# pj8912/python-p2p-network

Hardware: AMD Instinct MI355X
Metric: msg-edge relays/sec (GTEPS) at 10M peers x 4096 msgs; % HBM roofline (higher is better)
Workload: dtype u64

## Files before the change

python-p2p-network_amd/csrc/relay_kernels.hip:

```cpp
#include <hip/hip_runtime.h>

#include <algorithm>
#include <cstdlib>
#include <cstring>
#include <type_traits>

#include "device_util.h"

#ifndef P2PG_PICK_DIRECT
#define P2PG_PICK_DIRECT 1
#endif
#ifndef P2PG_PICK_FOLD
#define P2PG_PICK_FOLD 1
#endif


namespace p2pg {
namespace {

__global__ void k_zero_rows(uint64_t* plane, int32_t W, const int32_t* rows, int32_t n) {
  const int64_t i = (int64_t)blockIdx.x * blockDim.x + threadIdx.x;
  if (i >= (int64_t)n * W) return;
  const int64_t r = rows[i / W];
  if (r < 0) return;
  plane[r * W + (i % W)] = 0ull;
}

__global__ void k_seed(DevState st, const int32_t* src, int32_t M) {
  const int m = blockIdx.x * blockDim.x + threadIdx.x;
  if (m >= M) return;
  const int64_t v = src[m];
  if (v < 0) return;
  const uint64_t bit = 1ull << (m & 63);
  const int64_t o = v * st.W + (m >> 6);
  atomicOr((unsigned long long*)&st.F[0][o], (unsigned long long)bit);
  atomicOr((unsigned long long*)&st.seen[o], (unsigned long long)bit);
  atomicOr(&st.A[0][v >> 5], 1u << (v & 31));
  if (st.AW[0]) atomicOr((unsigned long long*)&st.AW[0][v], 1ull << (m >> 6));
}

template <bool CHURN, bool GOSSIP>
__global__ __launch_bounds__(256) void k_pull(DevGraph g, DevState st, RoundParams p) {
  const int lane = threadIdx.x & 63;
  const int wib = wave_in_block();
  const int64_t V = g.V;
  const int W = st.W;
  const int cur = p.round & 1, prv = cur ^ 1;
  const uint64_t* __restrict__ Src = GOSSIP ? st.E[prv] : st.F[prv];
  uint64_t* __restrict__ Fc = st.F[cur];
  const uint32_t* __restrict__ Ap = st.A[prv];
  const int64_t ntasks = (V + 31) >> 5;
  const int nslices = (W + 63) >> 6;
  uint64_t c[STAT_N] = {0, 0, 0, 0, 0, 0, 0, 0};

  for (int64_t task = (int64_t)blockIdx.x * WPB + wib; task < ntasks;
       task += (int64_t)gridDim.x * WPB) {
    const int64_t u0 = task << 5;
    const uint32_t sat0 = st.S[task];
    uint32_t sat = sat0;
    uint32_t todo = ~sat0 & phase_mask(p, task);
    if (V - u0 < 32) todo &= (1u << (V - u0)) - 1u;
    uint32_t aw = 0;
    while (todo) {
      const int b = __builtin_ctz(todo);
      todo &= todo - 1u;
      const int64_t u = u0 + b;
      const int64_t beg = g.rowptr[u], end = g.rowptr[u + 1];
      const uint64_t deg = (uint64_t)(end - beg);
      const uint64_t per_bit = GOSSIP ? (deg < (uint64_t)p.fanout ? deg : (uint64_t)p.fanout)
                                      : deg - 1;
      bool row_new = false, row_full = true;
      for (int sl = 0; sl < nslices; ++sl) {
        const int w = sl * 64 + lane;
        const bool valid = w < W;
        const uint64_t fm = valid ? full_mask(w, W, st.M) : 0ull;
        const uint64_t s = valid ? st.seen[u * W + w] : 0ull;
        const uint64_t need = fm & ~s;
        uint64_t acc = 0;
        if (__ballot(need != 0ull)) {
          for (int64_t cb = beg; cb < end; cb += 64) {
            const int64_t j = cb + lane;
            uint32_t srow = 0;
            bool act = false;
            if (j < end) {
              const int32_t v = g.colidx[j];
              act = bit_test(Ap, v);
              if (CHURN && act)
                act = !churn_dropped((uint32_t)(p.round - 1), gidx(g, u), gidx(g, v),
                                     p.churn_thr, p.cseed_lo, p.cseed_hi);
              srow = GOSSIP ? (uint32_t)j : (uint32_t)v;
            }
            uint64_t m = __ballot(act);
            while (m) {
              uint32_t sv[8];
              bool ok[8];
#pragma unroll
              for (int k = 0; k < 8; ++k) {
                ok[k] = m != 0ull;
                if (m) {
                  const int idx = __builtin_ctzll(m);
                  m &= m - 1ull;
                  sv[k] = (uint32_t)__builtin_amdgcn_readlane((int)srow, idx);
                } else {
                  sv[k] = 0u;
                }
              }
              uint64_t x[8];
#pragma unroll
              for (int k = 0; k < 8; ++k)
                x[k] = (ok[k] && need) ? Src[(int64_t)sv[k] * W + w] : 0ull;
#pragma unroll
              for (int k = 0; k < 8; ++k) acc |= x[k];
            }
          }
        }
        const uint64_t nw = acc & need;
        const bool any = __ballot(nw != 0ull) != 0ull;
        row_new |= any;
        if (__ballot(valid && (s | nw) != fm)) row_full = false;
        if (nw) st_prow(&st.seen[u * W + w], s | nw);
        if (valid && (any || nslices > 1)) st_prow(&Fc[u * W + w], nw);
        if (nw) {
          const uint64_t pc = (uint64_t)__popcll(nw);
          c[ST_NEW] += pc;
          c[ST_RELAYS] += pc * per_bit;
          c[ST_ACTIVE_W] += 1;
          c[ST_WEDGES] += deg;
        }
      }
      if (row_new) {
        aw |= 1u << b;
        if (lane == 0) {
          c[ST_ACTIVE_V] += 1;
          c[ST_DEG_ACT] += deg;
        }
      }
      if (row_full) sat |= 1u << b;
    }
    if (lane == 0) {
      put_active(st.A[cur], task, aw, p);
      if (sat != sat0) st.S[task] = sat;
    }
  }
  flush_stats(st.stats, c, lane);
}


struct PullStage {
  int b;
  int64_t beg, end;
  uint64_t s;
  int32_t v;
  uint32_t r;
  bool act;
  uint32_t aword;
  uint64_t mr;
  uint64_t am;
  uint32_t rv;
};

__device__ __forceinline__ bool aw_has(const uint64_t* __restrict__ AW, int64_t v, int w) {
  return !AW || ((ldc(AW + v) >> w) & 1ull);
}

struct FusedStage {
  int32_t u;
  uint32_t beg, end;
  uint64_t s;
  int32_t v;
  uint32_t aword;
  uint64_t mr;
  uint64_t am;
  uint32_t rv;
};

__device__ __forceinline__ uint64_t src_word(const uint64_t* __restrict__ Src, uint32_t row,
                                             int W, int lane, bool packed, uint64_t am,
                                             bool want) {
  if (!packed) return want ? at_row(Src, row, W)[lane] : 0ull;
  const bool here = want && ((am >> lane) & 1ull);
  const int pos = __popcll(am & ((1ull << lane) - 1ull));
  return here ? at_row(Src, row, W)[pos] : 0ull;
}


__device__ __forceinline__ uint64_t src_word_m(const uint64_t* __restrict__ Src, uint32_t row,
                                               int W, uint64_t am, uint64_t h) {
  uint64_t x = 0ull;
  if (__builtin_amdgcn_inverse_ballot_w64(h)) {
    const uint32_t pos = __builtin_amdgcn_mbcnt_hi((uint32_t)(am >> 32),
                                                   __builtin_amdgcn_mbcnt_lo((uint32_t)am, 0u));
#if P2PG_NT_LOADS
    x = __builtin_nontemporal_load(at_row(Src, row, W) + pos);
#else
    x = at_row(Src, row, W)[pos];
#endif
  }
  return x;
}

__device__ __forceinline__ uint64_t src_word_pair(const uint64_t* __restrict__ Src, uint32_t r0,
                                                  uint32_t r1, int W, uint32_t m0, uint32_t m1,
                                                  uint32_t h0, uint32_t h1) {
  uint64_t x = 0ull;
  if (__builtin_amdgcn_inverse_ballot_w64((uint64_t)h0 | ((uint64_t)h1 << 32))) {
    const bool lo = __builtin_amdgcn_mbcnt_hi(~0u, __builtin_amdgcn_mbcnt_lo(~0u, 0u)) < 32u;
    const uint32_t pos = __builtin_amdgcn_mbcnt_hi(m1, __builtin_amdgcn_mbcnt_lo(lo ? m0 : 0u, 0u));
    const uint32_t row = lo ? r0 : r1;
#if P2PG_NT_LOADS
    x = __builtin_nontemporal_load(at_row(Src, row, W) + pos);
#else
    x = at_row(Src, row, W)[pos];
#endif
  }
  return x;
}

template <bool CHURN, bool GOSSIP>
#ifndef P2PG_PULL_WAVES
#define P2PG_PULL_WAVES 1
#endif
__global__ __launch_bounds__(256, P2PG_PULL_WAVES) void k_pull1(DevGraph g, DevState st,
                                                                RoundParams p) {
  const int lane = threadIdx.x & 63;
  const int wib = wave_in_block();
  const int64_t V = g.V;
  const int W = st.W;
  const int cur = p.round & 1, prv = cur ^ 1;
  const uint64_t* __restrict__ Src = GOSSIP ? st.E[prv] : st.F[prv];
  uint64_t* __restrict__ Fc = st.F[cur];
  const uint32_t* __restrict__ Ap = st.A[prv];
  const uint64_t* __restrict__ AWp = GOSSIP ? st.AW[prv] : nullptr;
  const bool packed = GOSSIP && AWp != nullptr;
  const int64_t ntasks = (V + 31) >> 5;
  const bool valid = lane < W;
  const uint64_t fm = valid ? full_mask(lane, W, st.M) : 0ull;
  uint64_t c[STAT_N] = {0, 0, 0, 0, 0, 0, 0, 0};

  for (int64_t task = (int64_t)blockIdx.x * WPB + wib; task < ntasks;
       task += (int64_t)gridDim.x * WPB) {
    const int64_t u0 = task << 5;
    const uint32_t sat0 = st.S[task];
    uint32_t todo = ~sat0 & phase_mask(p, task);
    if (g.H) todo &= ~g.H[task];
    if (V - u0 < 32) todo &= (1u << (V - u0)) - 1u;
    if (!todo) {
      if (lane == 0 && p.phase != 1) st.A[cur][task] = 0u;
      continue;
    }
    int64_t rp = 0;
    if (lane <= 32 && u0 + lane <= V) rp = g.rowptr[u0 + lane];

    auto issue = [&](PullStage& q, int b) {
      q.b = b;
      q.act = false;
      q.v = 0;
      q.r = 0;
      q.s = 0;
      if (b < 0) return;
      q.beg = readlane64(rp, b);
      q.end = readlane64(rp, b + 1);
      if (valid) q.s = st.seen[(u0 + b) * W + lane];
      const int64_t j = q.beg + lane;
      if (j < q.end) {
        q.v = g.colidx[j];
        q.r = GOSSIP ? (uint32_t)j : (uint32_t)q.v;
      }
    };
    auto activity = [&](PullStage& q) {
      if (q.b < 0) return;
      const int64_t j = q.beg + lane;
      q.am = 0;
      q.aword = 0;
      if (j < q.end) {
        if (packed) q.am = AWp[q.v];
        q.aword = Ap[q.v >> 5];
      }
    };
    auto resolve = [&](PullStage& q) {
      const int64_t j = q.beg + lane;
      bool a = j < q.end && ((q.aword >> (q.v & 31)) & 1u);
      if (CHURN && a)
        a = !churn_dropped((uint32_t)(p.round - 1), gidx(g, u0 + q.b), gidx(g, q.v), p.churn_thr,
                           p.cseed_lo, p.cseed_hi);
      q.act = a;
    };
    auto next_bit = [](uint32_t& t) -> int {
      if (!t) return -1;
      const int b = __builtin_ctz(t);
      t &= t - 1u;
      return b;
    };

    uint32_t rest = todo;
    PullStage s1, s2, s3;
    issue(s1, next_bit(rest));
    issue(s2, next_bit(rest));
    activity(s1);
    uint32_t aw = 0, sat = sat0;
    while (s1.b >= 0) {
      issue(s3, next_bit(rest));
      activity(s2);
      const int64_t u = u0 + s1.b;
      const uint64_t deg = (uint64_t)(s1.end - s1.beg);
      const uint64_t need = fm & ~s1.s;
      uint64_t acc = 0;
      if (__ballot(need != 0ull)) {
        resolve(s1);
        uint64_t m = __ballot(s1.act);
        uint32_t srow = s1.r;
// ... 718 lines not shown
      uint64_t acc = 0;
      for (int64_t j = beg; j < end; ++j) {
        const int32_t v = g.colidx[j];
        if (!bit_test(Ap, v)) continue;
        if (FLOOD) {
          if (g.gone && g.gone[j]) continue;
          if (p.churn_thr && churn_dropped((uint32_t)(p.round - 1), gidx(g, u), gidx(g, v),
                                           p.churn_thr, p.cseed_lo, p.cseed_hi))
            continue;
          acc |= w < W ? Src[(int64_t)v * W + w] : 0ull;
        } else {
          acc |= packed ? src_word(Src, (uint32_t)j, W, lane, true, AWp[v], true)
                        : (w < W ? Src[j * W + w] : 0ull);
        }
      }
      if (acc) st.next[cur][u * W + w] |= acc;
      any |= __ballot(acc != 0ull) != 0ull;
    }
    if (any && lane == 0) atomicOr(&st.T[cur][u >> 5], 1u << (u & 31));
  }
}


#ifdef P2PG_PROF
#define PROF_DECL uint64_t pf_[9] = {0, 0, 0, 0, 0, 0, 0, 0, 0}; uint64_t pt_ = __builtin_amdgcn_s_memtime();
#define PROF_MARK(i)                                  \
  do {                                                \
    const uint64_t t_ = __builtin_amdgcn_s_memtime(); \
    pf_[i] += t_ - pt_;                               \
    pt_ = t_;                                         \
  } while (0)
#define PROF_FLUSH \
  if (lane == 0) for (int i_ = 0; i_ < 9; ++i_) atomicAdd(&st.prof[i_], (unsigned long long)pf_[i_]);
#define PROF_PARAMS , uint64_t* pf_, uint64_t& pt_
#define PROF_PASS , pf_, pt_
#else
#define PROF_DECL
#define PROF_MARK(i)
#define PROF_FLUSH
#define PROF_PARAMS
#define PROF_PASS
#endif

#ifndef P2PG_PICK_PAIRS
#define P2PG_PICK_PAIRS 0
#endif
#ifndef P2PG_COMPACT
#define P2PG_COMPACT 1
#endif

#ifndef P2PG_TBL_HALF_MAJOR
#define P2PG_TBL_HALF_MAJOR 1
#endif
struct ScatterLds {
  alignas(8) uint32_t tbl[GCHUNK * 128];
  uint16_t lst[GLIST];
};

__device__ __forceinline__ uint32_t tbl_ix(uint32_t j, uint32_t w, uint32_t h) {
#if P2PG_TBL_HALF_MAJOR
  return j * 128u + h * 64u + w;
#else
  return j * 128u + w * 2u + h;
#endif
}

__device__ __forceinline__ uint32_t tbl_entry_ix(uint32_t e) {
  return tbl_ix(0u, e >> 6, (e >> 5) & 1u);
}

__device__ __forceinline__ uint64_t tbl_word(const ScatterLds& L, int j, int w) {
#if P2PG_TBL_HALF_MAJOR
  return ((uint64_t)L.tbl[tbl_ix(j, w, 1)] << 32) | L.tbl[tbl_ix(j, w, 0)];
#else
  return *reinterpret_cast<const uint64_t*>(&L.tbl[tbl_ix(j, w, 0)]);
#endif
}

__device__ __forceinline__ void tbl_clear(ScatterLds& L, int j, int w) {
  L.tbl[tbl_ix(j, w, 0)] = 0u;
  L.tbl[tbl_ix(j, w, 1)] = 0u;
}

template <bool CHURN, int K, bool STORE_E, int PH = 0, bool PART = false, bool DIRECT = false, class CT>
__device__ __forceinline__ void scatter_row(const DevGraph& g, const DevState& st,
                                            const RoundParams& p, ScatterLds& L, int lane,
                                            int64_t v, int64_t rb, int64_t deg, int chunk,
                                            int sl, uint64_t f, uint32_t nbr, int nbr0,
                                            CT* c PROF_PARAMS) {
  const int W = st.W;
  const int cur = p.round & 1, nxt = cur ^ 1;
  uint64_t* __restrict__ nx = st.next[nxt];
  uint32_t* __restrict__ Tn = st.T[nxt];
  uint64_t* __restrict__ Eo = st.E[cur];
  const int k = K > 0 ? K : p.fanout;
  const int nb = chunk * GCHUNK;
  const int nn = (int)(deg - nb < GCHUNK ? deg - nb : GCHUNK);
  const bool all = deg <= k;
  const int w = sl * 64 + lane;
  const bool valid = w < W;
  const uint64_t fam = __ballot(f != 0ull);
  const bool anyf = fam != 0ull;
  if (!anyf && !STORE_E) return;
  const uint32_t gv = gidx_s(g, v);
  const PickKey pkey = pick_key((uint32_t)p.round, gv, p.gseed_lo, p.gseed_hi);

  auto one = [&](auto check_v, uint32_t e, bool ok) {
    constexpr bool CHECK = decltype(check_v)::value;
    const uint32_t wl = e >> 6, bit = e & 63u;
    const uint32_t mg = p.msg_base + (uint32_t)((sl * 64 + (int)wl) * 64) + bit;
    uint32_t* const col = &L.tbl[tbl_entry_ix(e)];
    const uint32_t mb = ok ? 1u << (bit & 31u) : 0u;
    uint32_t pk[K > 0 ? K : 1];
    if constexpr (P2PG_PICK_FOLD && K > 0 && K <= 4)
      gossip_picks_k<K>(pkey, mg, (uint32_t)deg, pk);
    else
      gossip_picks_t<(K > 0 ? K : 1)>((uint32_t)p.round, gv, mg, (uint32_t)deg, p.gseed_lo,
                                      p.gseed_hi, pk);
#pragma unroll
    for (int q = 0; q < (K > 0 ? K : 1); ++q) {
      const uint32_t jj = pk[q] - (uint32_t)nb;
      if (!CHECK || jj < (uint32_t)nn) atomicOr(col + jj * 128u, mb);
    }
  };
  auto pick_batch = [&](auto check_v, uint32_t n) {
    const uint32_t nbat = (n + 63) >> 6;
    const uint32_t i0 = (uint32_t)lane * nbat;
    const uint32_t cnt = i0 < n ? (n - i0 < nbat ? n - i0 : nbat) : 0u;
#if P2PG_PICK_PAIRS
    for (uint32_t b = 0; b < cnt; b += 2) {
      const uint32_t e0 = L.lst[i0 + b];
      const bool two = b + 1 < cnt;
      const uint32_t e1 = two ? L.lst[i0 + b + 1] : e0;
      one(check_v, e0, true);
      one(check_v, e1, two);
    }
#else
    uint32_t en = L.lst[i0];
    for (uint32_t b = 0; b < nbat; ++b) {
      const uint32_t e = en & 0x0FFFu;
      const uint32_t ni = i0 + b + 1;
      en = L.lst[ni < (uint32_t)GLIST ? ni : (uint32_t)GLIST - 1u];
      one(check_v, e, b < cnt);
    }
#endif
  };

  const int nf = __popcll(fam);
  const bool compact = P2PG_COMPACT && !CHURN && anyf && nf <= 32 &&
                       (STORE_E ? st.AW[cur] != nullptr : g.gone == nullptr);
  const bool use_tbl = anyf && !all;
  int seg = 64, rk_lane = 0, wc = 0, gl = 0;
  bool rk = false;
  if (compact) {
    seg = nf <= 16 ? 16 : 32;
    const int rank = (int)__builtin_amdgcn_mbcnt_hi(
        (uint32_t)(fam >> 32), __builtin_amdgcn_mbcnt_lo((uint32_t)fam, 0u));
    const int wr = __builtin_amdgcn_ds_permute((f ? rank : 63) << 2, lane);
    rk_lane = lane & (seg - 1);
    wc = __builtin_amdgcn_ds_bpermute(rk_lane << 2, wr);
    rk = rk_lane < nf;
    gl = lane / seg;
  }
  const int gper = 64 / seg;

  if (PH != 2 && use_tbl) {
    if (compact) {
      for (int j0 = 0; j0 < nn; j0 += gper) {
        const int jj = j0 + gl;
        if (rk && jj < nn) tbl_clear(L, jj, wc);
      }
    } else {
      for (int j = 0; j < nn; ++j) {
        tbl_clear(L, j, lane);
      }
    }
    const uint32_t cnt = (uint32_t)__popcll(f);
    bool direct = false;
    if constexpr (DIRECT && K > 0 && P2PG_PICK_DIRECT) {
      direct = __ballot(cnt > 1u) == 0ull;
      if (direct) {
        wave_lds_sync();
        const uint32_t e = ((uint32_t)lane << 6) | (uint32_t)__builtin_ctzll(f | (1ull << 63));
        if (nb == 0 && nn == (int)deg)
          one(std::false_type{}, e, f != 0ull);
        else
          one(std::true_type{}, e, f != 0ull);
        wave_lds_sync();
        PROF_MARK(7);
      }
    }
    const uint32_t incl = direct ? 0u : wave_scan_u32(cnt);
    const uint32_t total = direct ? 0u : (uint32_t)__builtin_amdgcn_readlane((int)incl, 63);
    const uint32_t pos0 = incl - cnt;
    constexpr uint32_t CAP = (uint32_t)GLIST - 1u;
    for (uint32_t lb = 0; lb < total; lb += CAP) {
      const uint32_t nw = total - lb < CAP ? total - lb : CAP;
      list_bits(L.lst, CAP, f, (uint32_t)lane << 6, pos0 - lb, nw);
      wave_lds_sync();
      PROF_MARK(6);
      const uint32_t n = nw;
      if constexpr (K > 0) {
        if (nb == 0 && nn == (int)deg)
          pick_batch(std::false_type{}, n);
        else
          pick_batch(std::true_type{}, n);
      } else {
        for (uint32_t i = lane; i < n; i += 64) {
          const uint32_t e = L.lst[i];
          const uint32_t wl = e >> 6, bit = e & 63u;
          const uint32_t mg = p.msg_base + (uint32_t)((sl * 64 + (int)wl) * 64) + bit;
          uint32_t* const col = &L.tbl[tbl_ix(0u, wl, bit >> 5)];
          const uint32_t mb = 1u << (bit & 31u);
          uint32_t pk[16];
          gossip_picks((uint32_t)p.round, gv, mg, (uint32_t)deg, k, p.gseed_lo, p.gseed_hi, pk);
          for (int q = 0; q < k; ++q) {
            const uint32_t jj = pk[q] - (uint32_t)nb;
            if (jj < (uint32_t)nn) atomicOr(col + jj * 128u, mb);
          }
        }
      }
      wave_lds_sync();
      PROF_MARK(7);
    }
  }
  if constexpr (PH == 1) return;
  if (compact) {
    const uint64_t segm = (1ull << seg) - 1ull;
    uint64_t fr = 0;
    if (all) {
      const uint32_t lo = (uint32_t)__builtin_amdgcn_ds_bpermute(wc << 2, (int)(uint32_t)f);
      const uint32_t hi = (uint32_t)__builtin_amdgcn_ds_bpermute(wc << 2, (int)(uint32_t)(f >> 32));
      fr = ((uint64_t)hi << 32) | lo;
    }
    for (int j0 = 0; j0 < nn; j0 += gper) {
      const int jj = j0 + gl;
      const bool ok = rk && jj < nn;
      uint64_t x = 0;
      if (ok) x = all ? fr : tbl_word(L, jj, wc);
      const uint32_t nj = (uint32_t)__builtin_amdgcn_ds_bpermute(
          (nbr0 + (jj < nn ? jj : 0)) << 2, (int)nbr);
      const uint64_t bal = __ballot(ok && x != 0ull);
      if (STORE_E && !(PART && (nj & REV_GHOST))) {
        if (ok) st_row(at_row(Eo, nj, W) + rk_lane, x);
      } else {
        const int64_t u = (int64_t)(PART ? nj & ~REV_GHOST : nj);
        if (x) atomicOr((unsigned long long*)at_row(nx, u, W) + sl * 64 + wc, (unsigned long long)x);
        if (rk_lane == 0 && ((bal >> (lane & ~(seg - 1))) & segm))
          atomicOr(&Tn[u >> 5], 1u << (u & 31));
      }
      if (lane == 0) c[ST_SCATTER] += (CT)__popcll(bal);
    }
    PROF_MARK(8);
    return;
  }
  auto tbl_row = [&](int j) -> uint64_t {
    return tbl_word(L, j, lane);
  };
  uint64_t xn = use_tbl && nn > 0 ? tbl_row(0) : 0ull;
  for (int j = 0; j < nn; ++j) {
    const uint64_t x = all ? f : xn;
    if (use_tbl && j + 1 < nn) xn = tbl_row(j + 1);
    const uint64_t bal = __ballot(x != 0ull);
    const uint32_t nj = (uint32_t)__builtin_amdgcn_readlane((int)nbr, nbr0 + j);
    if (STORE_E) {
      bool dropped = false;
      if (CHURN && bal)
        dropped = churn_dropped((uint32_t)p.round, gv, gidx_s(g, ldc(g.colidx + rb + nb + j)),
                                p.churn_thr, p.cseed_lo, p.cseed_hi);
      if (PART && (nj & REV_GHOST)) {
        const int64_t u = (int64_t)(nj & ~REV_GHOST);
        if (!dropped && bal) {
          if (x) atomicOr((unsigned long long*)at_row(nx, u, W) + w, (unsigned long long)x);
          if (lane == 0) {
            atomicOr(&Tn[u >> 5], 1u << (u & 31));
            c[ST_SCATTER] += (CT)__popcll(bal);
          }
        }
        continue;
      }
      if (st.AW[cur]) {
        if (f) st_row(at_row(Eo, nj, W) + __popcll(fam & ((1ull << lane) - 1ull)), dropped ? 0ull : x);
      } else if (valid) {
        st_row(at_row(Eo, nj, W) + w, dropped ? 0ull : x);
      }
      if (!dropped && lane == 0) c[ST_SCATTER] += (CT)__popcll(bal);
    } else {
      if (!bal) continue;
      if (g.gone && g.gone[rb + nb + j]) continue;
      const int64_t u = (int64_t)nj;
      if (CHURN && churn_dropped((uint32_t)p.round, gv, gidx_s(g, u), p.churn_thr,
                                 p.cseed_lo, p.cseed_hi))
        continue;
      if (x) atomicOr((unsigned long long*)at_row(nx, u, W) + w, (unsigned long long)x);
      if (lane == 0) {
        atomicOr(&Tn[u >> 5], 1u << (u & 31));
        c[ST_SCATTER] += (CT)__popcll(bal);
      }
    }
  }
  PROF_MARK(8);
}

template <bool CHURN, int K, bool STORE_E, bool PART = false>
__global__ __launch_bounds__(256) void k_gossip_scatter(DevGraph g, DevState st, RoundParams p,
                                                        const int64_t* __restrict__ hub_items,
                                                        int64_t n_hub, int64_t task0) {
  __shared__ ScatterLds lds[WPB];
  const int lane = threadIdx.x & 63;
  const int wib = wave_in_block();
  ScatterLds& L = lds[wib];
  const int64_t V = g.V;
  const int W = st.W;
  const int cur = p.round & 1;
  const uint64_t* __restrict__ Fc = st.F[cur];
  const uint64_t* __restrict__ AWc = W <= 64 ? st.AW[cur] : nullptr;
  const int64_t nwords = (V + 31) >> 5;
  const int64_t ntasks = nwords + ((n_hub + 63) >> 6);
  const int nslices = (W + 63) >> 6;
  uint64_t c[STAT_N] = {0, 0, 0, 0, 0, 0, 0, 0};
  PROF_DECL

  auto load_nbr = [&](int64_t rb, int nn) -> uint32_t {
    if (lane >= nn) return 0u;
    return STORE_E ? g.rev[rb + lane] : (uint32_t)g.colidx[rb + lane];
  };

  auto bitmap_task = [&](int64_t task, uint32_t todo) {
      const int64_t base = task << 5;
      auto pick_next = [&](uint32_t& t, int64_t& rb, int64_t& deg) -> int {
        while (t) {
          const int b = __builtin_ctz(t);
          t &= t - 1u;
          const int64_t vv = __builtin_amdgcn_readfirstlane((int)(base + b));
          rb = ldc(g.rowptr + vv);
          deg = ldc(g.rowptr + vv + 1) - rb;
          if (deg <= GCHUNK) return b;
        }
        return -1;
      };
      int64_t rb1 = 0, deg1 = 0, rb2 = 0, deg2 = 0;
      int b1 = pick_next(todo, rb1, deg1);
      uint64_t f1 = 0;
      uint32_t rv1 = 0;
      if (b1 >= 0) {
        if (lane < W && aw_has(AWc, base + b1, lane)) f1 = Fc[(base + b1) * W + lane];
        rv1 = load_nbr(rb1, (int)deg1);
      }
      while (b1 >= 0) {
        const int b2 = pick_next(todo, rb2, deg2);
        uint64_t f2 = 0;
        uint32_t rv2 = 0;
        if (b2 >= 0) {
          if (lane < W && aw_has(AWc, base + b2, lane)) f2 = Fc[(base + b2) * W + lane];
          rv2 = load_nbr(rb2, (int)deg2);
        }
        scatter_row<CHURN, K, STORE_E, 0, PART>(g, st, p, L, lane, base + b1, rb1, deg1, 0, 0, f1, rv1, 0,
                                       c PROF_PASS);
        b1 = b2;
        rb1 = rb2;
        deg1 = deg2;
        f1 = f2;
        rv1 = rv2;
      }
  };
  int64_t first = task0;
  if (nslices == 1 && task0 < nwords) {
    const int64_t wave = (int64_t)blockIdx.x * WPB + wib, nwave = (int64_t)gridDim.x * WPB;
    for (int64_t tb = task0 + wave * SCAN_W; tb < nwords; tb += nwave * SCAN_W) {
      const int64_t tl = tb + lane;
      const uint32_t al = lane < SCAN_W && tl < nwords ? st.A[cur][tl] : 0u;
      uint64_t busy = __ballot(al != 0u);
      while (busy) {
        const int l = __builtin_ctzll(busy);
        busy &= busy - 1ull;
        bitmap_task(tb + l, (uint32_t)__builtin_amdgcn_readlane((int)al, l));
      }
    }
    first = nwords;
  }
  for (int64_t task = first + (int64_t)blockIdx.x * WPB + wib; task < ntasks;
       task += (int64_t)gridDim.x * WPB) {
    auto one_source = [&](int64_t v, int chunk) {
      const int64_t rb = g.rowptr[v];
      const int64_t deg = g.rowptr[v + 1] - rb;
      const int nb = chunk * GCHUNK;
      const int nn = (int)(deg - nb < GCHUNK ? deg - nb : GCHUNK);
      const uint32_t rv = load_nbr(rb + nb, nn);
      for (int sl = 0; sl < nslices; ++sl) {
        const int w = sl * 64 + lane;
        const uint64_t f = w < W && aw_has(AWc, v, w) ? Fc[v * W + w] : 0ull;
        scatter_row<CHURN, K, STORE_E, 0, PART>(g, st, p, L, lane, v, rb, deg, chunk, sl, f, rv, 0, c PROF_PASS);
      }
    };
    if (task < nwords) {
      uint32_t todo = st.A[cur][task];
      while (todo) {
        const int b = __builtin_ctz(todo);
        todo &= todo - 1u;
        const int64_t v = (task << 5) + b;
        if (g.rowptr[v + 1] - g.rowptr[v] > GCHUNK) continue;
        one_source(v, 0);
      }
      continue;
    }
    const int64_t i = (task - nwords) * 64 + lane;
    int64_t item = 0;
    bool act = false;
    if (i < n_hub) {
      item = hub_items[i];
      act = bit_test(st.A[cur], item >> 32);
    }
    uint64_t am = __ballot(act);
    while (am) {
      const int l = __builtin_ctzll(am);
      am &= am - 1ull;
      const int64_t it = readlane64(item, l);
      one_source(it >> 32, (int)(it & 0xFFFFFFFFll));
    }
  }
  flush_stats(st.stats, c, lane);
}

#ifndef P2PG_FG
#define P2PG_FG 8
#endif
constexpr int FG = P2PG_FG;



#ifndef P2PG_FUSED_WAVES
#define P2PG_FUSED_WAVES 3
#endif
template <bool CHURN, int K, int MODE = 0, bool HALF = false, bool PART = false>
__global__ __launch_bounds__(256, P2PG_FUSED_WAVES) void k_gossip_fused(DevGraph g, DevState st,
                                                                        RoundParams p) {
  constexpr bool PO = MODE == 1, UP = MODE == 2, PL = MODE == 3;
  constexpr bool GATHER = MODE == 0 || PL;
  static_assert(!(PART && UP), "no update+push pass on partitioned ranks");
  if (!PART) g.gid = nullptr;
  g.gone = nullptr;
  g.gdeg = g.gpos = nullptr;
  __shared__ ScatterLds lds[WPB];
  const int lane = threadIdx.x & 63;
  const int wib = wave_in_block();
  const int64_t V = g.V;
  const int W = st.W;
  const int cur = p.round & 1, prv = cur ^ 1;
  const uint64_t* __restrict__ Src = st.E[prv];
  uint64_t* __restrict__ Fc = st.F[cur];
  const uint32_t* __restrict__ Ap = st.A[prv];
  const uint64_t* __restrict__ AWp = st.AW[prv];
  const int64_t ntasks = (V + 31) >> 5;
  const bool valid = lane < W;
  const uint64_t fm = valid ? full_mask(lane, W, st.M) : 0ull;
  uint32_t tot[STAT_N] = {0, 0, 0, 0, 0, 0, 0, 0};
  PROF_DECL

  const int64_t tstride = (int64_t)gridDim.x * WPB;
  int64_t pf_task = (int64_t)blockIdx.x * WPB + wib;
  uint32_t pf_s = 0, pf_h = 0;
  uint32_t pf_rp = 0;
  auto prefetch = [&](int64_t t) {
    pf_task = t;
    if (t < 0) return;
    pf_s = PO ? st.A[cur][t] : UP ? st.T[cur][t] : st.S[t];
    pf_h = g.H ? g.H[t] : 0u;
    const int64_t u0 = t << 5;
    pf_rp = (lane <= 32 && u0 + lane <= V) ? (uint32_t)g.rowptr[u0 + lane] : 0u;
  };
  if (pf_task >= ntasks) pf_task = -1;
  prefetch(pf_task);
  int32_t it_u0 = 0;
  uint32_t it_rest = 0;
  uint32_t rp = 0;
  auto next_peer = [&](uint32_t& beg, uint32_t& end) -> int32_t {
    while (!it_rest) {
      const int64_t t = pf_task;
      if (t < 0) return -1;
      const int64_t u0 = t << 5;
      const uint32_t sw = (uint32_t)__builtin_amdgcn_readfirstlane((int)pf_s);
      const uint32_t hw = (uint32_t)__builtin_amdgcn_readfirstlane((int)pf_h);
      uint32_t todo = (PO || UP ? sw : ~sw) & ~hw;
      if (V - u0 < 32) todo &= (1u << (V - u0)) - 1u;
      if (UP && lane == 0 && (sw & ~hw)) st.T[cur][t] = sw & hw;
      rp = pf_rp;
      prefetch(t + tstride < ntasks ? t + tstride : -1);
      if (!todo) {
        if (!PO && lane == 0) st.A[cur][t] = 0u;
        continue;
      }
      it_u0 = (int32_t)u0;
      it_rest = todo;
    }
    const int b = __builtin_ctz(it_rest);
    it_rest &= it_rest - 1u;
    beg = (uint32_t)__builtin_amdgcn_readlane((int)rp, b);
    end = (uint32_t)__builtin_amdgcn_readlane((int)rp, b + 1);
    return it_u0 + b;
  };

  auto issue = [&](FusedStage& q) {
    q.v = 0;
    q.rv = 0;
    q.s = 0;
    q.u = next_peer(q.beg, q.end);
    if (q.u < 0) return;
    if (valid) q.s = ld_once(at_row(PO ? Fc : st.seen, q.u, W) + lane);
    if (UP) q.am = valid ? at_row(st.next[cur], q.u, W)[lane] : 0ull;
    if (PO) q.am = ldc(st.AW[cur] + q.u);
    const uint32_t j = q.beg + lane;
    if (j < q.end) {
      if (GATHER) q.v = ld_once(&g.colidx[j]);
      if (!PL || PART) q.rv = ld_once(&g.rev[j]);
    }
  };
  auto activity = [&](FusedStage& q) {
    if (!GATHER || q.u < 0) return;
    const uint32_t j = q.beg + lane;
    q.am = 0;
    q.aword = 0;
    if (j < q.end) {
      q.am = AWp[q.v];
      q.aword = Ap[q.v >> 5];
    }
  };

  uint64_t X[FG];
  auto gather = [&](const FusedStage& q, uint64_t& mr) {
    if (!GATHER) {
#pragma unroll
      for (int k = 0; k < FG; ++k) X[k] = 0ull;
      mr = 0;
      return;
    }
    const uint64_t needm = __ballot((fm & ~q.s) != 0ull);
    const uint32_t jq = q.beg + lane;
    uint64_t m = __ballot(jq < q.end && ((q.aword >> (q.v & 31)) & 1u) &&
                          !(PART && (q.rv & REV_GHOST)));
    if constexpr (HALF) {
      constexpr int FH = FG / 2;
      uint32_t r0[FH], r1[FH], m0[FH], m1[FH];
#pragma unroll
      for (int k = FH; k < FG; ++k) X[k] = 0ull;
#pragma unroll
      for (int k = 0; k < FH; ++k) {
        r0[k] = r1[k] = m0[k] = m1[k] = 0u;
        if (m) {
          const int i0 = __builtin_ctzll(m);
          m &= ~(1ull << i0);
          r0[k] = q.beg + (uint32_t)i0;
          m0[k] = (uint32_t)__builtin_amdgcn_readlane((int)(uint32_t)q.am, i0);
        }
        if (m) {
          const int i1 = __builtin_ctzll(m);
          m &= ~(1ull << i1);
          r1[k] = q.beg + (uint32_t)i1;
          m1[k] = (uint32_t)__builtin_amdgcn_readlane((int)(uint32_t)q.am, i1);
        }
      }
#pragma unroll
      for (int k = 0; k < FH; ++k)
        X[k] = src_word_pair(Src, r0[k], r1[k], W, m0[k], m1[k], m0[k] & (uint32_t)needm,
                             m1[k] & (uint32_t)needm);
      mr = m;
      return;
    }
    uint32_t sv[FG];
    uint64_t am[FG];
#pragma unroll
    for (int k = 0; k < FG; ++k) {
      sv[k] = 0u;
      am[k] = 0ull;
      if (m) {
        const int idx = __builtin_ctzll(m);
        m &= ~(1ull << idx);
        sv[k] = q.beg + (uint32_t)idx;
        am[k] = (uint64_t)readlane64((int64_t)q.am, idx);
      }
    }
#pragma unroll
    for (int k = 0; k < FG; ++k) X[k] = src_word_m(Src, sv[k], W, am[k], am[k] & needm);
    mr = m;
  };

  uint32_t c[STAT_N] = {0, 0, 0, 0, 0, 0, 0, 0};
  int64_t ct = -1;
  uint32_t aw = 0, nsat = 0;
  auto finish_task = [&]() {
    if (ct < 0) return;
    if (!PO && lane == 0) {
      st.A[cur][ct] = aw;
      if (nsat) atomicOr(&st.S[ct], nsat);
    }
#pragma unroll
    for (int q = 0; q < STAT_N; ++q) {
      if (q == ST_ACTIVE_V) continue;
      const uint32_t r = wave_reduce_u32<false>(c[q]);
      c[q] = 0;
      if (q == ST_ACTIVE_W) {
        tot[ST_ACTIVE_W] += r & 0xFFFFu;
        tot[ST_ACTIVE_V] += r >> 16;
      } else {
        tot[q] += r;
      }
    }
    aw = 0;
    nsat = 0;
  };

  bool pend = false;
  int64_t pu = 0, pbeg = 0, pdeg = 0;
  uint64_t pnw = 0;
  uint32_t prcv = 0;
  auto flush_pending = [&]() {
    if (pend) {
      scatter_row<CHURN, K, true, 2, PART>(g, st, p, lds[wib], lane, pu, pbeg, pdeg, 0, 0, pnw, prcv,
                                     0, c PROF_PASS);
      pend = false;
    }
  };
  FusedStage sA, sB, sC, sD;
  issue(sA);
  issue(sB);
  activity(sA);
  if (sA.u >= 0) gather(sA, sA.mr);
  activity(sB);
  issue(sC);
  PROF_MARK(5);

  auto step = [&](FusedStage& a, FusedStage& b, FusedStage& cc, FusedStage& d) {
    const int64_t u = a.u;
    if ((u >> 5) != ct) {
      finish_task();
      ct = u >> 5;
    }
    const uint64_t deg = (uint64_t)(a.end - a.beg);
    const uint64_t need = PO ? ~0ull : fm & ~a.s;
    const uint64_t needm = __ballot(need != 0ull);
    uint64_t acc = 0;
#pragma unroll
    for (int k = 0; k < FG; ++k) acc |= X[k];
    if (UP) acc = a.am;
    uint64_t remote = 0;
    if (PART && GATHER && ((ldc(st.T[cur] + (u >> 5)) >> (u & 31)) & 1u) && valid)
      remote = ld_once(at_row(st.next[cur], u, W) + lane);
    PROF_MARK(0);
    if (GATHER) {
      uint64_t m = a.mr;
      uint64_t sam = a.am;
      uint32_t cb = a.beg;
      for (;;) {
        while (HALF && m) {
          uint32_t r0[4], r1[4], m0[4], m1[4];
#pragma unroll
          for (int k = 0; k < 4; ++k) {
            r0[k] = r1[k] = m0[k] = m1[k] = 0u;
            if (m) {
              const int i0 = __builtin_ctzll(m);
              m &= ~(1ull << i0);
              r0[k] = cb + (uint32_t)i0;
              m0[k] = (uint32_t)__builtin_amdgcn_readlane((int)(uint32_t)sam, i0);
            }
            if (m) {
              const int i1 = __builtin_ctzll(m);
              m &= ~(1ull << i1);
              r1[k] = cb + (uint32_t)i1;
              m1[k] = (uint32_t)__builtin_amdgcn_readlane((int)(uint32_t)sam, i1);
            }
          }
          uint64_t x[4];
#pragma unroll
          for (int k = 0; k < 4; ++k)
            x[k] = src_word_pair(Src, r0[k], r1[k], W, m0[k], m1[k], m0[k] & (uint32_t)needm,
                                 m1[k] & (uint32_t)needm);
#pragma unroll
          for (int k = 0; k < 4; ++k) acc |= x[k];
        }
        while (!HALF && m) {
          uint32_t sv[8];
          uint64_t am[8];
#pragma unroll
          for (int k = 0; k < 8; ++k) {
            am[k] = 0ull;
            if (m) {
              const int idx = __builtin_ctzll(m);
              m &= ~(1ull << idx);
              sv[k] = cb + (uint32_t)idx;
              am[k] = (uint64_t)readlane64((int64_t)sam, idx);
            } else {
              sv[k] = 0u;
            }
          }
          uint64_t x[8];
#pragma unroll
          for (int k = 0; k < 8; ++k)
            x[k] = src_word_m(Src, sv[k], W, am[k], am[k] & needm);
#pragma unroll
          for (int k = 0; k < 8; ++k) acc |= x[k];
        }
        cb += 64;
        if (cb >= a.end) break;
        const uint32_t j = cb + lane;
        bool act = false;
        sam = 0;
        if (j < a.end) {
          const int32_t v = g.colidx[j];
          act = bit_test(Ap, v) && !(PART && (g.rev[j] & REV_GHOST));
          if (act) sam = AWp[v];
        }
        m = __ballot(act);
      }
    }
    __builtin_amdgcn_s_waitcnt(0x0F70);
    PROF_MARK(1);
    if (HALF) acc |= bperm64(lane ^ 32, acc);
    if (PART) acc |= remote;
    if (UP && acc) {
      st_prow(at_row(st.next[cur], u, W) + lane, 0ull);
      c[ST_AUX] += 1;
    }
    flush_pending();
    if (b.u >= 0) gather(b, b.mr);
    activity(cc);
    issue(d);
    PROF_MARK(2);
    const uint64_t nw = PO ? ((a.am >> lane) & 1ull ? a.s : 0ull) : acc & need;
    const uint64_t wm = __ballot(nw != 0ull);
    if (!PO && nw) {
      st_frow(at_row(st.seen, u, W) + lane, a.s | nw);
      const uint32_t pc = (uint32_t)__popcll(nw);
      const uint32_t kf = K > 0 ? (uint32_t)K : (uint32_t)p.fanout;
      const uint32_t per_bit = deg < (uint64_t)kf ? (uint32_t)deg : kf;
      c[ST_NEW] += pc;
      c[ST_RELAYS] += pc * per_bit;
      c[ST_ACTIVE_W] += 1;
      c[ST_WEDGES] += (uint32_t)deg;
    }
    if (wm) {
      if (!PO) {
        if (valid && p.store_f && (p.store_f != 2 || nw)) st_frow(at_row(Fc, u, W) + lane, nw);
        aw |= 1u << (u & 31);
        if (lane == 0) {
          st.AW[cur][u] = wm;
          c[ST_ACTIVE_W] += 1u << 16;
          c[ST_DEG_ACT] += (uint32_t)deg;
        }
      }
      if (PL) {
      } else if (deg <= (uint64_t)GCHUNK) {
        scatter_row<CHURN, K, true, 1, PART, PO || UP>(g, st, p, lds[wib], lane, u, a.beg, (int64_t)deg, 0, 0,
                                       nw, a.rv, 0, c PROF_PASS);
        pend = true;
        pu = u;
        pbeg = a.beg;
        pdeg = (int64_t)deg;
        pnw = nw;
        prcv = a.rv;
      } else if (deg <= 64) {
        for (int ch = 0; (int64_t)ch * GCHUNK < (int64_t)deg; ++ch)
          scatter_row<CHURN, K, true, 0, PART, PO || UP>(g, st, p, lds[wib], lane, u, a.beg, (int64_t)deg, ch, 0,
                                      nw, a.rv, ch * GCHUNK, c PROF_PASS);
      } else {
        for (int ch = 0; (int64_t)ch * GCHUNK < (int64_t)deg; ++ch) {
          const int off = (ch * GCHUNK) & 63;
          const uint32_t j = a.beg + (uint32_t)(ch * GCHUNK - off) + lane;
          const uint32_t rvb = j < a.end ? g.rev[j] : 0u;
          __builtin_amdgcn_s_waitcnt(0x0F70);
          scatter_row<CHURN, K, true, 0, PART, PO || UP>(g, st, p, lds[wib], lane, u, a.beg, (int64_t)deg, ch, 0,
                                      nw, rvb, off, c PROF_PASS);
        }
      }
    }
    PROF_MARK(3);
    if (!PO && !__ballot(valid && (a.s | nw) != fm)) nsat |= 1u << (u & 31);
  };
  for (;;) {
    if (sA.u < 0) break;
    step(sA, sB, sC, sD);
    if (sB.u < 0) break;
    step(sB, sC, sD, sA);
    if (sC.u < 0) break;
    step(sC, sD, sA, sB);
    if (sD.u < 0) break;
    step(sD, sA, sB, sC);
  }
  flush_pending();
  finish_task();
  PROF_MARK(4);
  PROF_FLUSH
  if (lane == 0) {
    unsigned long long* shard = st.stats + (blockIdx.x & (STAT_SHARDS - 1)) * STAT_N;
#pragma unroll
    for (int q = 0; q < STAT_N; ++q)
      if (tot[q]) atomicAdd(shard + q, (unsigned long long)tot[q]);
  }
}

__device__ int32_t find_parent(const DevGraph& g, const DevState& st, const RoundParams& p,
                               int64_t u, int m) {
  const int prv = (p.round & 1) ^ 1;
  const int W = st.W;
  const uint64_t bit = 1ull << (m & 63);
  const int w = m >> 6;
  const int64_t beg = g.rowptr[u], end = g.rowptr[u + 1];
  for (int64_t e = beg; e < end; ++e) {
    const int32_t v = g.colidx[e];
    if (g.gone && g.gone[e]) continue;
    if (!bit_test(st.A[prv], v)) continue;
    if (!(st.F[prv][(int64_t)v * W + w] & bit)) continue;
    if (p.churn_thr && churn_dropped((uint32_t)(p.round - 1), gidx(g, u), gidx(g, v),
                                     p.churn_thr, p.cseed_lo, p.cseed_hi))
      continue;
    if (p.mode == 1) {
      const int64_t vb = g.rowptr[v];
      const bool ghost = g.gpos && g.gpos[e] >= 0;
      const int64_t dv = ghost ? (int64_t)g.gdeg[v] : g.rowptr[v + 1] - vb;
      if (dv > p.fanout) {
        int64_t lo = 0, hi = dv;
        if (ghost) {
          lo = g.gpos[e];
        } else {
          while (lo < hi) {
            const int64_t mid = (lo + hi) >> 1;
            if (g.colidx[vb + mid] < u) lo = mid + 1; else hi = mid;
          }
        }
        uint32_t pk[16];
        gossip_picks((uint32_t)(p.round - 1), gidx(g, v), p.msg_base + (uint32_t)m,
                     (uint32_t)dv, p.fanout, p.gseed_lo, p.gseed_hi, pk);
        bool hit = false;
        for (int q = 0; q < p.fanout; ++q) hit |= (pk[q] == (uint32_t)lo);
        if (!hit) continue;
      }
    }
    return v;
  }
  return -2;
}

__global__ __launch_bounds__(256) void k_record(DevGraph g, DevState st, RoundParams p) {
  const int lane = threadIdx.x & 63;
  const int wib = wave_in_block();
  const int cur = p.round & 1;
  const int W = st.W;
  const int64_t ntasks = (g.V + 31) >> 5;
  const int nslices = (W + 63) >> 6;
  for (int64_t task = (int64_t)blockIdx.x * WPB + wib; task < ntasks;
       task += (int64_t)gridDim.x * WPB) {
    uint32_t aw = st.A[cur][task];
    while (aw) {
      const int b = __builtin_ctz(aw);
      aw &= aw - 1u;
      const int64_t u = (task << 5) + b;
      for (int sl = 0; sl < nslices; ++sl) {
        const int w = sl * 64 + lane;
        uint64_t f = w < W ? st.F[cur][u * W + w] : 0ull;
        while (f) {
          const int bit = __builtin_ctzll(f);
          f &= f - 1ull;
          const int m = w * 64 + bit;
          st.hop[u * st.M + m] = p.round;
          const int32_t par = p.round == 0 ? -1 : find_parent(g, st, p, u, m);
          st.parent[u * st.M + m] = par < 0 ? -1 : par;
        }
      }
    }
  }
}

__global__ __launch_bounds__(256) void k_deliveries(DevGraph g, DevState st, RoundParams p,
                                                    int64_t cap, int32_t* peer, int32_t* msg,
                                                    int32_t* parent,
                                                    unsigned long long* counter) {
  const int lane = threadIdx.x & 63;
  const int wib = wave_in_block();
  const int cur = p.round & 1;
  const int W = st.W;
  const int64_t ntasks = (g.V + 31) >> 5;
  const int nslices = (W + 63) >> 6;
  for (int64_t task = (int64_t)blockIdx.x * WPB + wib; task < ntasks;
       task += (int64_t)gridDim.x * WPB) {
    uint32_t aw = st.A[cur][task];
    while (aw) {
      const int b = __builtin_ctz(aw);
      aw &= aw - 1u;
      const int64_t u = (task << 5) + b;
      for (int sl = 0; sl < nslices; ++sl) {
        const int w = sl * 64 + lane;
        uint64_t f = w < W ? st.F[cur][u * W + w] : 0ull;
        while (f) {
          const int bit = __builtin_ctzll(f);
          f &= f - 1ull;
          const int m = w * 64 + bit;
          const unsigned long long pos = atomicAdd(counter, 1ull);
          if ((int64_t)pos < cap) {
            peer[pos] = (int32_t)u;
            msg[pos] = m;
            const int32_t par = p.round == 0 ? -1 : find_parent(g, st, p, u, m);
            parent[pos] = par < 0 ? -1 : par;
          }
        }
      }
    }
  }
}

__global__ __launch_bounds__(256) void k_pack(DevState st, int plane, int round,
                                              const int32_t* __restrict__ ids, int64_t n,
                                              uint64_t* __restrict__ out) {
  const int lane = threadIdx.x & 63;
  const int W = st.W;
  const int64_t nw = (int64_t)gridDim.x * WPB;
  for (int64_t i = (int64_t)blockIdx.x * WPB + wave_in_block(); i < n; i += nw) {
    const int64_t v = ids[i];
    if (plane == 0) {
      const bool act = bit_test(st.A[round & 1], v);
      for (int w = lane; w < W; w += 64) out[i * W + w] = act ? st.F[round & 1][v * W + w] : 0ull;
    } else {
      uint64_t* nx = st.next[(round + 1) & 1];
      for (int w = lane; w < W; w += 64) {
        out[i * W + w] = nx[v * W + w];
        nx[v * W + w] = 0ull;
      }
      if (lane == 0) atomicAnd(&st.T[(round + 1) & 1][v >> 5], ~(1u << (v & 31)));
    }
  }
}

__global__ __launch_bounds__(256) void k_unpack(DevState st, int plane, int round,
                                                const int32_t* __restrict__ ids, int64_t n,
                                                const uint64_t* __restrict__ in) {
  const int lane = threadIdx.x & 63;
  const int W = st.W;
  const int64_t nw = (int64_t)gridDim.x * WPB;
  for (int64_t i = (int64_t)blockIdx.x * WPB + wave_in_block(); i < n; i += nw) {
    const int64_t v = ids[i];
    bool any = false;
    for (int w = lane; w < W; w += 64) {
      const uint64_t x = in[i * W + w];
      any |= x != 0ull;
      if (plane == 0) st.F[round & 1][v * W + w] = x;
      else if (x) atomicOr((unsigned long long*)&st.next[(round + 1) & 1][v * W + w], (unsigned long long)x);
    }
    if (__ballot(any) && lane == 0) {
      if (plane == 0) atomicOr(&st.A[round & 1][v >> 5], 1u << (v & 31));
      else atomicOr(&st.T[(round + 1) & 1][v >> 5], 1u << (v & 31));
    }
  }
}

__global__ __launch_bounds__(256) void k_pack_live(DevState st, int plane, int round,
                                                   const int32_t* __restrict__ ids, int64_t n,
                                                   const int64_t* __restrict__ seg_off, int nseg,
                                                   unsigned long long* __restrict__ seg_cnt,
                                                   int64_t* __restrict__ out) {
  const int lane = threadIdx.x & 63;
  const int W = st.W;
  const int64_t R = 1 + W;
  const int64_t nwaves = (int64_t)gridDim.x * WPB;
  uint64_t* __restrict__ src = plane == 0 ? st.F[round & 1] : st.next[(round + 1) & 1];
  uint32_t* __restrict__ bits = plane == 0 ? st.A[round & 1] : st.T[(round + 1) & 1];
  for (int64_t base = ((int64_t)blockIdx.x * WPB + wave_in_block()) * 64; base < n; base += nwaves * 64) {
    const int64_t i = base + lane;
    const bool valid = i < n;
    const int64_t v = valid ? ids[i] : 0;
    const bool live = valid && bit_test(bits, v);
    int seg = 0;
    for (int q = 1; q < nseg; ++q) seg += i >= ldc(seg_off + q);
    int64_t pos = 0;
    uint64_t todo = __ballot(live);
    while (todo) {
      const int q0 = __builtin_amdgcn_readlane(seg, __builtin_ctzll(todo));
      const uint64_t m = __ballot(live && seg == q0);
      unsigned long long b0 = 0;
      if (lane == 0) b0 = atomicAdd(&seg_cnt[q0], (unsigned long long)__popcll(m));
      b0 = (unsigned long long)readlane64((int64_t)b0, 0);
      if (live && seg == q0)
        pos = (int64_t)b0 + __builtin_amdgcn_mbcnt_hi((uint32_t)(m >> 32), __builtin_amdgcn_mbcnt_lo((uint32_t)m, 0u));
      todo &= ~m;
    }
    uint64_t lv = __ballot(live);
    while (lv) {
      const int l = __builtin_ctzll(lv);
      lv &= lv - 1ull;
      const int64_t vl = readlane64(v, l);
      const int sq = __builtin_amdgcn_readlane(seg, l);
      const int64_t rec = (ldc(seg_off + sq) + readlane64(pos, l)) * R;
      if (lane == 0) out[rec] = readlane64(i, l) - ldc(seg_off + sq);
      for (int w = lane; w < W; w += 64) {
        out[rec + 1 + w] = (int64_t)src[vl * W + w];
        if (plane == 1) src[vl * W + w] = 0ull;
      }
      if (plane == 1 && lane == 0) atomicAnd(&bits[vl >> 5], ~(1u << (vl & 31)));
    }
  }
}

struct RecOffsets {
  int64_t off[P2PG_MAX_RANKS + 1];
};

__global__ __launch_bounds__(256) void k_unpack_live(DevState st, int plane, int round,
                                                     const int32_t* __restrict__ ids,
                                                     const int64_t* __restrict__ list_off, int nseg,
                                                     RecOffsets ro, const int64_t* __restrict__ in) {
  const int lane = threadIdx.x & 63;
  const int W = st.W;
  const int64_t R = 1 + W;
  const int64_t nrec = ro.off[nseg];
  for (int64_t i = (int64_t)blockIdx.x * WPB + wave_in_block(); i < nrec; i += (int64_t)gridDim.x * WPB) {
    int p = 0;
    for (int q = 1; q < nseg; ++q) p += i >= ro.off[q];
    const int64_t idx = ldc(in + i * R);
    if (idx < 0 || idx >= ldc(list_off + p + 1) - ldc(list_off + p)) continue;
    const int64_t v = ids[ldc(list_off + p) + idx];
    for (int w = lane; w < W; w += 64) {
      const uint64_t x = (uint64_t)in[i * R + 1 + w];
      if (plane == 0) st.F[round & 1][v * W + w] = x;
      else if (x) atomicOr((unsigned long long*)&st.next[(round + 1) & 1][v * W + w], (unsigned long long)x);
    }
    if (lane == 0) {
      if (plane == 0) atomicOr(&st.A[round & 1][v >> 5], 1u << (v & 31));
      else atomicOr(&st.T[(round + 1) & 1][v >> 5], 1u << (v & 31));
    }
  }
}

__global__ void k_column(const uint64_t* __restrict__ plane, int32_t W, int32_t w, int64_t V,
                         uint64_t* __restrict__ out) {
  for (int64_t v = (int64_t)blockIdx.x * blockDim.x + threadIdx.x; v < V;
       v += (int64_t)gridDim.x * blockDim.x)
    out[v] = plane[v * W + w];
}

__global__ void k_philox(int32_t n, const uint32_t* ctr, uint32_t k0, uint32_t k1,
                         uint32_t* out) {
  const int i = blockIdx.x * blockDim.x + threadIdx.x;
  if (i >= n) return;
  u32x4 c = {ctr[4 * i], ctr[4 * i + 1], ctr[4 * i + 2], ctr[4 * i + 3]};
  u32x4 r = philox4x32_10(c, k0, k1);
  out[4 * i] = r.x;
  out[4 * i + 1] = r.y;
  out[4 * i + 2] = r.z;
  out[4 * i + 3] = r.w;
}

}

hipError_t launch_zero_rows(uint64_t* plane, int32_t W, const int32_t* rows, int32_t n,
                            hipStream_t s) {
  const int64_t tot = (int64_t)n * W;
  if (tot == 0) return hipSuccess;
  hipLaunchKernelGGL(k_zero_rows, dim3((unsigned)((tot + 255) / 256)), dim3(256), 0, s, plane,
                     W, rows, n);
  return hipGetLastError();
}

hipError_t launch_seed(const DevState& st, const int32_t* src, int32_t M, hipStream_t s) {
  if (M == 0) return hipSuccess;
  hipLaunchKernelGGL(k_seed, dim3((M + 255) / 256), dim3(256), 0, s, st, src, M);
// ... 471 lines not shown
```

Before: 420.2.

## Add wide-pass scatter path for high-degree peers using LDS mask table

Adds a scatter_wide routine for peers whose degree exceeds GCHUNK. It processes connections in groups of 64, builds per-connection, per-rank bitmasks in an LDS table via atomicOr, then flushes whole 64-bit words with plain stores instead of global atomics. It also marks the low-degree branch as likely. The aim is to replace many global atomicOr operations on E rows with coalesced stores. In exchange it adds extra passes, LDS clearing and wave syncs, and it is only used for non-churn, compile-time-fanout, non-partitioned variants.

```diff
diff --git a/python-p2p-network_amd/csrc/pass_plan.h b/python-p2p-network_amd/csrc/pass_plan.h
--- /dev/null
+++ b/python-p2p-network_amd/csrc/pass_plan.h
@@ -0,0 +1,47 @@
+#pragma once
+#include <cstdint>
+
+#if defined(__HIPCC__) || defined(__CUDACC__)
+#define PASS_PLAN_HD __host__ __device__ inline
+#else
+#define PASS_PLAN_HD inline
+#endif
+
+constexpr int PLAN_CELLS = 2048;
+constexpr int PLAN_MASKS = PLAN_CELLS / 2;
+constexpr int PLAN_GROUP = 64;
+
+PASS_PLAN_HD int plan_groups(int deg) { return (deg + PLAN_GROUP - 1) / PLAN_GROUP; }
+PASS_PLAN_HD int plan_group_begin(int g) { return g * PLAN_GROUP; }
+PASS_PLAN_HD int plan_group_conns(int deg, int g) {
+  const int c = deg - g * PLAN_GROUP;
+  return c < PLAN_GROUP ? c : PLAN_GROUP;
+}
+
+PASS_PLAN_HD int plan_pass_words(int conns) { return conns <= 16 ? 64 : conns <= 32 ? 32 : 16; }
+
+PASS_PLAN_HD int plan_passes(int conns, int nactive) {
+  const int wp = plan_pass_words(conns);
+  return (nactive + wp - 1) / wp;
+}
+PASS_PLAN_HD int plan_pass_rank0(int conns, int p) { return p * plan_pass_words(conns); }
+PASS_PLAN_HD int plan_pass_ranks(int conns, int nactive, int p) {
+  const int wp = plan_pass_words(conns);
+  const int r = nactive - p * wp;
+  return r < wp ? r : wp;
+}
+
+PASS_PLAN_HD int plan_seg(int ranks) { return ranks <= 16 ? 16 : ranks <= 32 ? 32 : 64; }
+PASS_PLAN_HD int plan_pass_cells(int conns, int ranks) { return conns * plan_seg(ranks) * 2; }
+PASS_PLAN_HD int plan_flush_count(int conns, int ranks) {
+  const int per = 64 / plan_seg(ranks);
+  return (conns + per - 1) / per;
+}
+
+PASS_PLAN_HD uint64_t plan_rank_words(uint64_t fam, int rank0, int ranks) {
+  uint64_t out = 0;
+  int r = 0;
+  for (uint64_t m = fam; m; m &= m - 1, ++r)
+    if (r >= rank0 && r < rank0 + ranks) out |= m & (~m + 1);
+  return out;
+}
diff --git a/python-p2p-network_amd/csrc/relay_kernels.hip b/python-p2p-network_amd/csrc/relay_kernels.hip
--- a/python-p2p-network_amd/csrc/relay_kernels.hip
+++ b/python-p2p-network_amd/csrc/relay_kernels.hip
@@ -6,6 +6,7 @@
 #include <type_traits>
 
 #include "device_util.h"
+#include "pass_plan.h"
 
 #ifndef P2PG_PICK_DIRECT
 #define P2PG_PICK_DIRECT 1
@@ -1330,6 +1331,108 @@
   PROF_MARK(8);
 }
 
+#ifndef P2PG_WIDE_PASS
+#define P2PG_WIDE_PASS 1
+#endif
+template <int K, class CT>
+__device__ __forceinline__ void scatter_wide(const DevGraph& g, const DevState& st,
+                                             const RoundParams& p, ScatterLds& L, int lane,
+                                             int64_t v, uint32_t beg, uint32_t deg, uint64_t f,
+                                             uint32_t rv0, CT* c PROF_PARAMS) {
+  static_assert(K > 0, "compile-time fanout only");
+  static_assert(GCHUNK * 128 >= PLAN_CELLS, "the pass plan's table");
+  const int W = st.W;
+  uint64_t* __restrict__ Eo = st.E[p.round & 1];
+  const uint64_t fam = __ballot(f != 0ull);
+  const int nf = __popcll(fam);
+  const uint32_t gv = gidx_s(g, v);
+  const PickKey pkey = pick_key((uint32_t)p.round, gv, p.gseed_lo, p.gseed_hi);
+  const uint32_t cnt = (uint32_t)__popcll(f);
+  const uint32_t incl = wave_scan_u32(cnt);
+  const uint32_t total = (uint32_t)__builtin_amdgcn_readlane((int)incl, 63);
+  const uint32_t pos0 = incl - cnt;
+  const int rank = (int)__builtin_amdgcn_mbcnt_hi((uint32_t)(fam >> 32),
+                                                  __builtin_amdgcn_mbcnt_lo((uint32_t)fam, 0u));
+  const uint32_t rpos = (uint32_t)__builtin_amdgcn_ds_permute((f ? rank : 63) << 2, (int)pos0);
+  constexpr uint32_t CAP = (uint32_t)GLIST - 1u;
+  uint32_t have = ~0u;
+  const bool check = deg > (uint32_t)PLAN_GROUP;
+
+  for (uint32_t cb = 0; cb < deg; cb += PLAN_GROUP) {
+    const int C = (int)(deg - cb < (uint32_t)PLAN_GROUP ? deg - cb : (uint32_t)PLAN_GROUP);
+    uint32_t rv = rv0;
+    if (cb) {
+      const uint32_t j = beg + cb + (uint32_t)lane;
+      rv = j < beg + deg ? g.rev[j] : 0u;
+      __builtin_amdgcn_s_waitcnt(0x0F70);
+    }
+    const int wp = plan_pass_words(C);
+    const uint32_t Cc = check ? (uint32_t)C : ~0u;
+    for (int r0 = 0; r0 < nf; r0 += wp) {
+      const int nr = nf - r0 < wp ? nf - r0 : wp;
+      const int seg = plan_seg(nr);
+      const int nmask = C * seg;
+      uint64_t* const tb = reinterpret_cast<uint64_t*>(L.tbl);
+      for (int i = lane; i < nmask; i += 64) tb[i] = 0ull;
+      const uint32_t s = (uint32_t)__builtin_amdgcn_readlane((int)rpos, r0);
+      const uint32_t e = r0 + nr < nf ? (uint32_t)__builtin_amdgcn_readlane((int)rpos, r0 + nr) : total;
+      for (uint32_t lb = 0; lb < e; lb += CAP) {
+        if (lb + CAP <= s) continue;
+        if (lb != have) {
+          wave_lds_sync();
+          list_bits(L.lst, CAP, f, (uint32_t)lane << 6, pos0 - lb, total - lb < CAP ? total - lb : CAP);
+          have = lb;
+        }
+        wave_lds_sync();
+        PROF_MARK(6);
+        const uint32_t a = (s > lb ? s : lb) - lb;
+        const uint32_t n = (e < lb + CAP ? e : lb + CAP) - lb - a;
+        const uint32_t nbat = (n + 63) >> 6;
+        const uint32_t i0 = (uint32_t)lane * nbat;
+        const uint32_t mine = i0 < n ? (n - i0 < nbat ? n - i0 : nbat) : 0u;
+        auto at = [&](uint32_t i) { return a + i < (uint32_t)GLIST ? a + i : (uint32_t)GLIST - 1u; };
+        uint32_t en = L.lst[at(i0)];
+        for (uint32_t b = 0; b < nbat; ++b) {
+          const uint32_t ent = en & 0x0FFFu;
+          en = L.lst[at(i0 + b + 1)];
+          const uint32_t wl = ent >> 6, bit = ent & 63u;
+          const uint32_t mg = p.msg_base + wl * 64u + bit;
+          const uint32_t rr = ((uint32_t)__popcll(fam & ((1ull << wl) - 1ull)) - (uint32_t)r0) &
+                              (uint32_t)(seg - 1);
+          uint32_t* const col = &L.tbl[rr * 2u + (bit >> 5)];
+          const uint32_t mb = b < mine ? 1u << (bit & 31u) : 0u;
+          uint32_t pk[K];
+          if constexpr (P2PG_PICK_FOLD && K <= 4)
+            gossip_picks_k<K>(pkey, mg, deg, pk);
+          else
+            gossip_picks_t<K>((uint32_t)p.round, gv, mg, deg, p.gseed_lo, p.gseed_hi, pk);
+#pragma unroll
+          for (int q = 0; q < K; ++q) {
+            const uint32_t jj = pk[q] - cb;
+            if (jj < Cc) atomicOr(col + jj * (uint32_t)(seg * 2), mb);
+          }
+        }
+        wave_lds_sync();
+        PROF_MARK(7);
+      }
+      const int rk_lane = lane & (seg - 1);
+      const int gl = lane / seg;
+      const int gper = 64 / seg;
+      for (int j0 = 0; j0 < C; j0 += gper) {
+        const int jj = j0 + gl;
+        const bool ok = rk_lane < nr && jj < C;
+        const uint64_t x = ok ? tb[j0 * seg + lane] : 0ull;
+        const uint32_t nj = (uint32_t)__builtin_amdgcn_ds_bpermute((jj < C ? jj : 0) << 2, (int)rv);
+        const uint64_t bal = __ballot(x != 0ull);
+        if (ok) st_row(at_row(Eo, nj, W) + r0 + rk_lane, x);
+        if (lane == 0) c[ST_SCATTER] += (CT)__popcll(bal);
+      }
+      wave_lds_sync();
+      PROF_MARK(8);
+    }
+  }
+}
+
 template <bool CHURN, int K, bool STORE_E, bool PART = false>
 __global__ __launch_bounds__(256) void k_gossip_scatter(DevGraph g, DevState st, RoundParams p,
                                                         const int64_t* __restrict__ hub_items,
@@ -1776,7 +1879,7 @@
         }
       }
       if (PL) {
-      } else if (deg <= (uint64_t)GCHUNK) {
+      } else if (__builtin_expect(deg <= (uint64_t)GCHUNK, 1)) {
         scatter_row<CHURN, K, true, 1, PART, PO || UP>(g, st, p, lds[wib], lane, u, a.beg, (int64_t)deg, 0, 0,
                                        nw, a.rv, 0, c PROF_PASS);
         pend = true;
@@ -1785,6 +1888,8 @@
         pdeg = (int64_t)deg;
         pnw = nw;
         prcv = a.rv;
+      } else if constexpr (P2PG_WIDE_PASS && !CHURN && K > 0 && !PART) {
+        scatter_wide<K>(g, st, p, lds[wib], lane, u, a.beg, (uint32_t)deg, nw, a.rv, c PROF_PASS);
       } else if (deg <= 64) {
         for (int ch = 0; (int64_t)ch * GCHUNK < (int64_t)deg; ++ch)
           scatter_row<CHURN, K, true, 0, PART, PO || UP>(g, st, p, lds[wib], lane, u, a.beg, (int64_t)deg, ch, 0,
```

Measured after the change: 430.1 (median of 6 runs). +2.3%, better.
